# JuliaGaussianProcesses/ApproximateGPs.jl

Hardware: AMD Instinct MI355X
Metric: SVGP ELBO evals/sec at N=1e6, M=1024 (higher is better)
Workload: dtype f64

## Files before the change

### approximategps.jl_amd/csrc/device_common.hpp

```cpp
#pragma once
#include <hip/hip_runtime.h>
#include <type_traits>
#include <utility>

#include "diag.hpp"
#include <stdint.h>

#include <mutex>
#include <string>
#include <vector>

namespace svgp {

inline std::string& note_text() { static thread_local std::string s; return s; }
inline void leave_note(const std::string& s) {
  if (note_text().size() < 2048) note_text() += (note_text().empty() ? "" : "; ") + s;
}
inline std::string take_note() {
  std::string s;
  s.swap(note_text());
  return s;
}

inline void set_max_lds(const void* fn, hipFuncAttribute attr, int bytes) {
// ... 530 lines not shown
#endif
  using LdsP = const volatile __attribute__((address_space(3))) T*;
  struct RFrag { LdsP a, b0, b1; };
  static __device__ __forceinline__ LdsP lds_opaque(const T* p) {
    uint32_t v = uint32_t(uintptr_t((const __attribute__((address_space(3))) T*)(p)));
    asm("" : "+v"(v));
    return (LdsP)(uintptr_t(v));
  }
  static __device__ __forceinline__ RFrag rfrag(const T* smem) {
    const AFrag fr = afrag(smem);
    return RFrag{lds_opaque(fr.a), lds_opaque(fr.b0), lds_opaque(fr.b1)};
  }
  static constexpr int kMaxRotImmP = ((NBUF - 1) * PA_TILE + (kPairP ? 3 * 2 * PPP : 3 * 4 * PLD) + (MI - 1) * 32) * int(sizeof(T));
  static constexpr int kMaxRotImmQ = ((NBUF - 1) * QA_TILE + 3 * QSLAB + (NJ - 2) * 16) * int(sizeof(T));
  static_assert(!kAsync || (kMaxRotImmP < 65536 && kMaxRotImmQ < 65536), "a fragment read's offset must fit the ds_read immediate");
  template <int B, int KSLAB, int ILO = 0, int IHI = MI - 1>
  static __device__ __forceinline__ void load_rfrag(Frag& f, const RFrag& fr) {
    constexpr int AOFF = B * PA_TILE + (kPairP ? KSLAB * 2 * PPP : KSLAB * 4 * PLD);
    constexpr int QOFF = B * QA_TILE + KSLAB * QSLAB;
#pragma unroll
    for (int i = 0; i < MI; ++i)
      if (i >= ILO && i <= IHI) f.a[i] = fr.a[AOFF + i * 32];
    if (ILO <= IHI) {
      static_assert(NJ % 2 == 0, "column tiles come in even / odd pairs");
      static_assert(QR == 2 || NJ == 2, "the quad image is written for two column tiles per wave");
#pragma unroll
      for (int j = 0; j < NJ; j += 2) {
        f.b[j] = fr.b0[QOFF + j * 16];
        f.b[j + 1] = fr.b1[QOFF + j * 16];
      }
    }
  }
  struct ADst { uint32_t p, q; };
  static __device__ __forceinline__ ADst a_dst(const T* smem, int wv) {
    const uint32_t l = uint32_t(uintptr_t((const __attribute__((address_space(3))) T*)(smem)));
    return ADst{l + uint32_t(wv * (kPairP ? PPP : PLD) * int(sizeof(T))),
                l + uint32_t((NBUF * PA_TILE + wv * QPP) * int(sizeof(T)))};
  }
  template <int IMM>
  static __device__ __forceinline__ void glds16_at(const void* sbase, uint32_t voff, uint32_t lds) {
    asm volatile("s_add_u32 m0, %0, %3\n\tglobal_load_lds_dwordx4 %1, %2" ::"s"(lds), "v"(voff), "s"(sbase), "n"(IMM) : "memory", "scc");
  }
  template <int B>
  static __device__ __forceinline__ void dma_tile_at(const T* __restrict__ psrc, const T* __restrict__ qsrc, const AOff& off,
                                                     const ADst& dst) {
    if constexpr (!diag::ablate<1>) dma_rows<B * PA_TILE, NW * (kPairP ? PPP : PLD)>(psrc, off.p, dst.p, std::make_integer_sequence<int, DP>{});
    if constexpr (!diag::ablate<2>) dma_rows<B * QA_TILE, NW * QPP>(qsrc, off.q, dst.q, std::make_integer_sequence<int, DQ>{});
  }
  template <int BASE, int STRIDE, int N, int... Q>
  static __device__ __forceinline__ void dma_rows(const T* __restrict__ src, const uint32_t (&voff)[N], uint32_t dst,
                                                  std::integer_sequence<int, Q...>) {
    (glds16_at<(BASE + Q * STRIDE) * int(sizeof(T))>(src, voff[Q], dst), ...);
  }
  static constexpr int kAskT = -1;
  template <int B, int ILO, int IHI, int MORE = kAskT, typename QSrc, typename WSrc>
  static __device__ __forceinline__ void rstep(Acc& acc, Frag (&f)[2], const T* __restrict__ Pbase, int64_t pstride,
                                               const AOff& off, int t, int nsteps, QSrc& qsrc, WSrc& wsrc, T* __restrict__ smem,
                                               const ADst& dst, const RFrag& fr) {
    constexpr int KS = BK / 4;
    constexpr bool W = WSrc::on;
    constexpr int PER_TILE = DMA_PER_TILE + (W ? 1 : 0);
    constexpr int BN = (B + 1) % NBUF;
    static_assert(KS == 4, "written for 16-deep steps");
    static_assert(B >= 0 && B < NBUF, "buffer index");
    T* Ws = smem + NBUF * (PA_TILE + QA_TILE);
    const T* wl = Ws + B * W_TILE + ((threadIdx.x & 63) >> 4);
    load_rfrag<B, 1, ILO, IHI>(f[1], fr);
    mma_frag<ILO, IHI>(acc, f[0]);
    scale_b<1, W>(f[1], wl);
    load_rfrag<B, 2, ILO, IHI>(f[0], fr);
    mma_frag<ILO, IHI>(acc, f[1]);
    scale_b<2, W>(f[0], wl);
    load_rfrag<B, 3, ILO, IHI>(f[1], fr);
    mma_frag<ILO, IHI>(acc, f[0]);
    scale_b<3, W>(f[1], wl);
    const bool more1 = (MORE == kAskT) ? (t + 1 < nsteps) : (MORE >= 1);
    const bool more2 = (MORE == kAskT) ? (t + 2 < nsteps) : (MORE >= 2);
    const bool more3 = (MORE == kAskT) ? (t + 3 < nsteps) : (MORE >= 3);
    if (more1) {
      if (more2) wait_barrier<PER_TILE>();
      else wait_barrier<0>();
      load_rfrag<BN, 0>(f[0], fr);
      scale_b<0, W>(f[0], Ws + BN * W_TILE + ((threadIdx.x & 63) >> 4));
      if (more3) {
        dma_tile_at<B>(Pbase + int64_t(t + 3) * pstride, qsrc(t + 3), off, dst);
        if constexpr (W) dma_w(wsrc(t + 3), Ws + B * W_TILE);
      }
    }
    mma_frag<ILO, IHI>(acc, f[1]);
  }
#ifndef SVGP_WSTEP
#define SVGP_WSTEP 0
#endif
  struct WRegs { T w[4]; };
  static __device__ __forceinline__ void load_w(WRegs& wr, const T* __restrict__ wl) {
#pragma unroll
    for (int q = 0; q < 4; ++q) wr.w[q] = wl[q * 4];
  }
  template <int KSLAB>
  static __device__ __forceinline__ void scale_bw(Frag& f, const WRegs& wr) {
#pragma unroll
    for (int j = 0; j < NJ; ++j) f.b[j] *= wr.w[KSLAB];
  }
  template <typename QSrc, typename WSrc>
  static __device__ __forceinline__ void astep_w(Acc& acc, Frag (&f)[2], WRegs& wr, const T* __restrict__ Pbase, int64_t pstride,
                                                 const AOff& off, int t, int nsteps, QSrc& qsrc, WSrc& wsrc, T* __restrict__ smem,
                                                 int& b, const AFrag& fr) {
    constexpr int PER_TILE = DMA_PER_TILE + 1;
    static_assert(BK / 4 == 4, "written for 16-deep steps");
    const T* fa = fr.a + b * PA_TILE;
    const T* fb0 = fr.b0 + b * QA_TILE;
    const T* fb1 = fr.b1 + b * QA_TILE;
    T* Ws = smem + NBUF * (PA_TILE + QA_TILE);
    load_afrag<1>(f[1], fa, fb0, fb1);
    mma_frag(acc, f[0]);
    scale_bw<1>(f[1], wr);
    load_afrag<2>(f[0], fa, fb0, fb1);
    mma_frag(acc, f[1]);
    scale_bw<2>(f[0], wr);
    load_afrag<3>(f[1], fa, fb0, fb1);
    mma_frag(acc, f[0]);
    scale_bw<3>(f[1], wr);
    if (t + 1 < nsteps) {
      if (t + 2 < nsteps) wait_barrier<PER_TILE>();
      else wait_barrier<0>();
      const int bn = (b + 1 == NBUF) ? 0 : b + 1;
      load_w(wr, Ws + bn * W_TILE + ((threadIdx.x & 63) >> 4));
      load_afrag<0>(f[0], fr.a + bn * PA_TILE, fr.b0 + bn * QA_TILE, fr.b1 + bn * QA_TILE);
      if (t + 3 < nsteps) {
        dma_tile(Pbase + int64_t(t + 3) * pstride, qsrc(t + 3), off, smem + b * PA_TILE, smem + NBUF * PA_TILE + b * QA_TILE);
        dma_w(wsrc(t + 3), Ws + b * W_TILE);
      }
      b = bn;
      mma_frag(acc, f[1]);
#ifndef SVGP_WSTEP
#define SVGP_WSTEP 1
#endif
#if SVGP_WSTEP == 1
      __builtin_amdgcn_sched_barrier(0);
#endif
      scale_bw<0>(f[0], wr);
    } else {
      mma_frag(acc, f[1]);
    }
  }
#define SVGP_ASTEP(LO, HI, TT) astep<LO, HI>(acc, f, Pbase, pstride, off, (TT), nsteps, qsrc, wsrc, smem, b, fr)
#define SVGP_RSTEP(B, LO, HI, TT, ...) rstep<B, LO, HI, ##__VA_ARGS__>(acc, f, Pbase, pstride, off, (TT), nsteps, qsrc, wsrc, smem, dst, fr)
  template <int TRI, typename QSrc>
  static __device__ __forceinline__ void loop_tri_async(Acc& acc, const T* __restrict__ Pbase, int64_t ldp, int nsteps,
                                                        QSrc&& qsrc, T* __restrict__ smem, int64_t ldq = NT) {
    NoWeights nw;
    loop_tri_async_w<TRI>(acc, Pbase, ldp, nsteps, qsrc, nw, smem, ldq);
  }
  template <int TRI, typename QSrc, typename WSrc>
  static __device__ __forceinline__ void loop_tri_async_w(Acc& acc, const T* __restrict__ Pbase, int64_t ldp, int nsteps,
                                                          QSrc&& qsrc, WSrc&& wsrc, T* __restrict__ smem, int64_t ldq = NT) {
    if (nsteps <= 0) return;
    constexpr int ND = NB / BK;
    constexpr bool W = std::remove_reference_t<WSrc>::on;
    constexpr int PER_TILE = DMA_PER_TILE + (W ? 1 : 0);
    static_assert(TRI == 0 || (ND == 8 && MI == 4), "triangular steps are written out for BK = 16, 128-row panels");
    const AOff off = a_offsets(ldp, ldq);
    const int64_t pstride = int64_t(BK) * ldp;
    const int nreg = (TRI > 0) ? nsteps - ND : nsteps;
    Frag f[2];
    constexpr bool kTwin = W && TRI == 0 && SVGP_WSTEP != 0;
    if constexpr (SVGP_ASYNC_ROT && !kTwin) {
      constexpr bool kRemFirst = TRI >= 0;
      const int rem = kRemFirst ? nreg % NBUF : 0;
      const int s0 = (rem == 0) ? 0 : NBUF - rem, s1 = (s0 + 1 == NBUF) ? 0 : s0 + 1, s2 = (s1 + 1 == NBUF) ? 0 : s1 + 1;
      const ADst dst = a_dst(smem, wave_index());
      auto displaced = [&](int sb) { return ADst{dst.p + uint32_t(sb * PA_TILE * int(sizeof(T))), dst.q + uint32_t(sb * QA_TILE * int(sizeof(T)))}; };
      T* Ws = smem + NBUF * (PA_TILE + QA_TILE);
      dma_tile_at<0>(Pbase, qsrc(0), off, displaced(s0));
      if constexpr (W) dma_w(wsrc(0), Ws + s0 * W_TILE);
      if (nsteps > 1) {
        dma_tile_at<0>(Pbase + pstride, qsrc(1), off, displaced(s1));
        if constexpr (W) dma_w(wsrc(1), Ws + s1 * W_TILE);
      }
      if (nsteps > 2) {
        dma_tile_at<0>(Pbase + 2 * pstride, qsrc(2), off, displaced(s2));
        if constexpr (W) dma_w(wsrc(2), Ws + s2 * W_TILE);
      }
      if (nsteps > 2) wait_barrier<2 * PER_TILE>();
      else if (nsteps > 1) wait_barrier<PER_TILE>();
      else wait_barrier<0>();
      const RFrag fr = rfrag(smem);
      const T* wl0 = Ws + ((threadIdx.x & 63) >> 4);
      if constexpr (kRemFirst) {
        int zt = 0;
        asm volatile("" : "+s"(zt));
        int t = rem;
        if (rem == 0) {
          load_rfrag<0, 0>(f[0], fr);
          scale_b<0, W>(f[0], wl0);
        } else if (rem == 1) {
          load_rfrag<2, 0>(f[0], fr);
          scale_b<0, W>(f[0], wl0 + 2 * W_TILE);
          SVGP_RSTEP(2, 0, MI - 1, zt);
        } else {
          load_rfrag<1, 0>(f[0], fr);
          scale_b<0, W>(f[0], wl0 + W_TILE);
          SVGP_RSTEP(1, 0, MI - 1, zt); SVGP_RSTEP(2, 0, MI - 1, zt + 1);
        }
        for (; t < nreg; t += 3) {
          SVGP_RSTEP(0, 0, MI - 1, t); SVGP_RSTEP(1, 0, MI - 1, t + 1); SVGP_RSTEP(2, 0, MI - 1, t + 2);
        }
        if constexpr (TRI > 0) {
          SVGP_RSTEP(0, 0, 3, t + 0, 3); SVGP_RSTEP(1, 0, 3, t + 1, 3); SVGP_RSTEP(2, 1, 3, t + 2, 3); SVGP_RSTEP(0, 1, 3, t + 3, 3);
          SVGP_RSTEP(1, 2, 3, t + 4, 3); SVGP_RSTEP(2, 2, 3, t + 5, 2); SVGP_RSTEP(0, 3, 3, t + 6, 1); SVGP_RSTEP(1, 3, 3, t + 7, 0);
        }
      } else {
        load_rfrag<0, 0>(f[0], fr);
        scale_b<0, W>(f[0], wl0);
        SVGP_RSTEP(0, 0, 0, 0); SVGP_RSTEP(1, 0, 0, 1); SVGP_RSTEP(2, 0, 1, 2); SVGP_RSTEP(0, 0, 1, 3);
        SVGP_RSTEP(1, 0, 2, 4); SVGP_RSTEP(2, 0, 2, 5); SVGP_RSTEP(0, 0, 3, 6); SVGP_RSTEP(1, 0, 3, 7);
        constexpr int B0 = ND % NBUF, B1 = (B0 + 1) % NBUF, B2 = (B0 + 2) % NBUF;
        int t = ND;
        for (; t + 2 < nreg; t += 3) {
          SVGP_RSTEP(B0, 0, MI - 1, t); SVGP_RSTEP(B1, 0, MI - 1, t + 1); SVGP_RSTEP(B2, 0, MI - 1, t + 2);
        }
        if (t < nreg) SVGP_RSTEP(B0, 0, MI - 1, t);
        if (t + 1 < nreg) SVGP_RSTEP(B1, 0, MI - 1, t + 1);
      }
      __builtin_amdgcn_sched_barrier(0);
    } else {
      const AFrag fr = afrag(smem);
      T* Qs = smem + NBUF * PA_TILE;
      T* Ws = smem + NBUF * (PA_TILE + QA_TILE);
      dma_tile(Pbase, qsrc(0), off, smem, Qs);
      if constexpr (W) dma_w(wsrc(0), Ws);
      if (nsteps > 1) {
        dma_tile(Pbase + pstride, qsrc(1), off, smem + PA_TILE, Qs + QA_TILE);
        if constexpr (W) dma_w(wsrc(1), Ws + W_TILE);
      }
      if (nsteps > 2) {
        dma_tile(Pbase + 2 * pstride, qsrc(2), off, smem + 2 * PA_TILE, Qs + 2 * QA_TILE);
        if constexpr (W) dma_w(wsrc(2), Ws + 2 * W_TILE);
      }
      if (nsteps > 2) wait_barrier<2 * PER_TILE>();
      else if (nsteps > 1) wait_barrier<PER_TILE>();
      else wait_barrier<0>();
      load_afrag<0>(f[0], fr.a, fr.b0, fr.b1);
      scale_b<0, W>(f[0], Ws + ((threadIdx.x & 63) >> 4));
      int b = 0, t = 0;
      if (TRI < 0) {
        SVGP_ASTEP(0, 0, 0); SVGP_ASTEP(0, 0, 1); SVGP_ASTEP(0, 1, 2); SVGP_ASTEP(0, 1, 3);
        SVGP_ASTEP(0, 2, 4); SVGP_ASTEP(0, 2, 5); SVGP_ASTEP(0, 3, 6); SVGP_ASTEP(0, 3, 7);
        t = ND;
      }
      if constexpr (kTwin) {
        WRegs wr;
        load_w(wr, Ws + ((threadIdx.x & 63) >> 4));
        for (; t < nreg; ++t) astep_w(acc, f, wr, Pbase, pstride, off, t, nsteps, qsrc, wsrc, smem, b, fr);
      } else {
        for (; t < nreg; ++t) astep<0, MI - 1>(acc, f, Pbase, pstride, off, t, nsteps, qsrc, wsrc, smem, b, fr);
      }
      if (TRI > 0) {
        SVGP_ASTEP(0, 3, nreg + 0); SVGP_ASTEP(0, 3, nreg + 1); SVGP_ASTEP(1, 3, nreg + 2); SVGP_ASTEP(1, 3, nreg + 3);
        SVGP_ASTEP(2, 3, nreg + 4); SVGP_ASTEP(2, 3, nreg + 5); SVGP_ASTEP(3, 3, nreg + 6); SVGP_ASTEP(3, 3, nreg + 7);
      }
    }
    __syncthreads();
  }
#undef SVGP_RSTEP
#undef SVGP_ASTEP
};

}
```

### approximategps.jl_amd/csrc/diag.hpp

```cpp
#pragma once
#include <hip/hip_runtime.h>

namespace svgp {
namespace diag {
#ifdef SVGP_ABLATE
constexpr int kAblate = SVGP_ABLATE;
#else
constexpr int kAblate = 0;
#endif
template <int BIT>
inline constexpr bool ablate = (kAblate & BIT) != 0;
}
}

#if defined(SVGP_STRIP_STAMPS) && defined(SVGP_DIAG_TU_STRIP)
namespace svgp {
__device__ unsigned long long g_strip_stamps[128];
__shared__ unsigned long long s_strip_stamps[128];
__device__ unsigned long long g_wg_times[16][12];
}
extern "C" int svgp_debug_strip_stamps(unsigned long long* out) {
  return int(hipMemcpyFromSymbol(out, HIP_SYMBOL(svgp::g_strip_stamps), sizeof(svgp::g_strip_stamps)));
}
extern "C" int svgp_debug_wg_times(unsigned long long* out) {
  return int(hipMemcpyFromSymbol(out, HIP_SYMBOL(svgp::g_wg_times), sizeof(svgp::g_wg_times)));
}
#define SVGP_SSTAMP(i) do { if (stamping && threadIdx.x == 0) s_strip_stamps[i] += clock64(); } while (0)
#define SVGP_SSTAMP_KERNEL_BEGIN()                            \
  int strips_done = 0;                                        \
  if (threadIdx.x < 128) s_strip_stamps[threadIdx.x] = 0;     \
  __syncthreads()
#define SVGP_SSTAMP_STRIP_BEGIN()                                                                                          \
  const bool stamping = (blockIdx.x == 37 && strips_done >= 1);                                                            \
  if (stamping && threadIdx.x == 0) s_strip_stamps[127] += 1;                                                              \
  if (threadIdx.x == 0 && blockIdx.x % 37 == 0 && blockIdx.x / 37 < 16 && strips_done < 10)                                \
    g_wg_times[blockIdx.x / 37][strips_done] = clock64();                                                                  \
  ++strips_done
#define SVGP_SSTAMP_KERNEL_END()                                                                                           \
  do {                                                                                                                     \
    if (blockIdx.x == 37 && threadIdx.x < 128) g_strip_stamps[threadIdx.x] = s_strip_stamps[threadIdx.x];                  \
    if (threadIdx.x == 0 && blockIdx.x % 37 == 0 && blockIdx.x / 37 < 16) {                                                \
      g_wg_times[blockIdx.x / 37][10] = clock64();                                                                         \
      g_wg_times[blockIdx.x / 37][11] = (unsigned long long)(__builtin_amdgcn_s_getreg((20 << 0) | (0 << 6) | (3 << 11)) & 0xf) | \
                                        ((unsigned long long)strips_done << 8);                         \
      for (int q = strips_done; q < 10; ++q) g_wg_times[blockIdx.x / 37][q] = 0;                                           \
    }                                                                                                                      \
  } while (0)
#else
#define SVGP_SSTAMP(i)
#define SVGP_SSTAMP_KERNEL_BEGIN()
#define SVGP_SSTAMP_STRIP_BEGIN()
#define SVGP_SSTAMP_KERNEL_END()
#endif

#if defined(SVGP_POTF2_STAMPS) && defined(SVGP_DIAG_TU_PREP)
namespace svgp {
__device__ unsigned long long g_potf2_stamps[128];
}
extern "C" int svgp_debug_potf2_stamps(unsigned long long* out) {
  return int(hipMemcpyFromSymbol(out, HIP_SYMBOL(svgp::g_potf2_stamps), sizeof(svgp::g_potf2_stamps)));
}
#define SVGP_STAMP(i) do { if (threadIdx.x == 0) g_potf2_stamps[i] = clock64(); } while (0)
#define SVGP_STAMPW(i) do { if (threadIdx.x == 64) g_potf2_stamps[i] = clock64(); } while (0)
#else
#define SVGP_STAMP(i)
#define SVGP_STAMPW(i)
#endif
```

### approximategps.jl_amd/csrc/strip.hip

```cpp
#define SVGP_DIAG_TU_STRIP
#include "device_common.hpp"
#include "kernels.hpp"
#include "knobs.hpp"
#include "lik.hpp"

#ifndef SVGP_ASYNC
#define SVGP_ASYNC 1
#endif
#ifndef SVGP_TRI
#define SVGP_TRI 3
#endif

#include <cstdlib>
#include <type_traits>

namespace svgp {

namespace {

#ifndef SVGP_PREGEN_EXPTAB
#define SVGP_PREGEN_EXPTAB 1
#endif
template <typename T, int NT, int NTHR, int F, int DL>
__device__ __forceinline__ void pregen_mfma(const T* __restrict__ xs, const T* __restrict__ zs, int d, int64_t Mp, int64_t M,
                                            double variance_d, T* __restrict__ work, const double* __restrict__ exptab = nullptr) {
  constexpr int KS = DL / 4, JT = NT / 16, NW = NTHR / 64;
  constexpr bool XREG = (DL <= 16);
  using M16 = Mfma16<T>;
  using acc_t = typename M16::acc_t;
  const int lane = threadIdx.x & 63, wave = threadIdx.x >> 6, l15 = lane & 15, g = lane >> 4;
  const T variance = T(variance_d);
  const T c1 = (F == KSE) ? T(-0.5) : T(1);
  const T c0 = (F == KSE) ? T(log(variance_d)) : T(0);
  const T ascale = (F == KSE) ? T(1) : T(-2);
  T xb[XREG ? JT : 1][XREG ? KS : 1], xn[JT];
  const T* __restrict__ xl = xs + g * NT + l15;
#pragma unroll
  for (int jt = 0; jt < JT; ++jt) {
    T s = T(0);
#pragma unroll
    for (int q = 0; q < KS; ++q) {
      const T v = xl[(4 * q) * NT + jt * 16];
      if constexpr (XREG) xb[jt][q] = v;
      s = fma(v, v, s);
    }
    s += __shfl_xor(s, 16);
    s += __shfl_xor(s, 32);
    xn[jt] = fma(c1, s, c0);
  }
  for (int kb = wave; kb < int(Mp / 16); kb += NW) {
    const int64_t k0 = int64_t(kb) * 16;
    const bool inside = __builtin_amdgcn_readfirstlane(int(k0 + 16 <= M)) != 0;
    T za[KS];
    T s = T(0);
#pragma unroll
    for (int q = 0; q < KS; ++q) {
      const int f = 4 * q + g;
      const T v = (f < d) ? zs[int64_t(f) * Mp + k0 + l15] : T(0);
      za[q] = ascale * v;
      s = fma(v, v, s);
    }
    s += __shfl_xor(s, 16);
    s += __shfl_xor(s, 32);
    s *= c1;
    T zn[4];
#pragma unroll
    for (int r = 0; r < 4; ++r) zn[r] = __shfl(s, M16::row(lane, r));
#pragma unroll
    for (int jt = 0; jt < JT; ++jt) {
      acc_t acc;
#pragma unroll
      for (int r = 0; r < 4; ++r) acc[r] = xn[jt] + zn[r];
      if constexpr (XREG) {
#pragma unroll
        for (int q = 0; q < KS; ++q) acc = M16::mma(za[q], xb[jt][q], acc);
      } else {
        acc_t acc2 = {0, 0, 0, 0};
        __builtin_amdgcn_sched_barrier(0);
#pragma unroll
        for (int q = 0; q < KS; q += 2) {
          acc = M16::mma(za[q], xl[(4 * q) * NT + jt * 16], acc);
          acc2 = M16::mma(za[q + 1], xl[(4 * q + 4) * NT + jt * 16], acc2);
        }
#pragma unroll
        for (int r = 0; r < 4; ++r) acc[r] += acc2[r];
      }
      T out[4];
#pragma unroll
      for (int r = 0; r < 4; ++r) {
        const T v = acc[r];
        if constexpr (SVGP_PREGEN_EXPTAB && F == KSE && sizeof(T) == 8) out[r] = T(kexp_tab(double(v > c0 ? c0 : v), exptab));
        else out[r] = (F == KSE) ? kexp(v > c0 ? c0 : v) : kappa<T>(F, v < T(0) ? T(0) : v, variance);
      }
      if (inside) {
#pragma unroll
        for (int r = 0; r < 4; ++r) work[(k0 + M16::row(lane, r)) * NT + jt * 16 + l15] = out[r];
      } else {
#pragma unroll
        for (int r = 0; r < 4; ++r) {
          const int64_t k = k0 + M16::row(lane, r);
          work[k * NT + jt * 16 + l15] = (k < M) ? out[r] : T(0);
        }
        asm volatile("" ::: "memory");
      }
    }
  }
}


template <typename G, typename T, int NT, int NTHR>
__device__ __forceinline__ void store_tile_point_major(const typename G::Acc& acc, T* __restrict__ smem, T* __restrict__ out,
                                                       int64_t c0, int64_t Mp, int row0) {
  constexpr int HC = NT < 64 ? NT : 64, RS = G::NB + (sizeof(T) == 8 ? 4 : 8), VEC = G::VEC, CPR = G::NB / VEC;
  using V = typename G::V;
  static_assert(size_t(HC) * RS * sizeof(T) <= ((SVGP_ASYNC && G::kAsync) ? G::ASYNC_LDS_BYTES : G::LDS_BYTES),
                "the transposition tile must fit the staging buffers");
#pragma unroll
  for (int p = 0; p < NT / HC; ++p) {
#pragma unroll
    for (int j = 0; j < G::NJ; ++j) {
      const int col = G::acc_col(j);
      if (col / HC == p) {
#pragma unroll
        for (int i = 0; i < G::MI; ++i)
#pragma unroll
          for (int r = 0; r < 4; ++r) smem[(col % HC) * RS + G::acc_row(i, r)] = acc.v[i][j][r];
      }
    }
    __syncthreads();
    for (int e = threadIdx.x; e < HC * CPR; e += NTHR) {
      const int col = e / CPR, rv = (e % CPR) * VEC;
      *reinterpret_cast<V*>(out + (c0 + p * HC + col) * Mp + row0 + rv) = *reinterpret_cast<const V*>(smem + col * RS + rv);
    }
    __syncthreads();
  }
}

#ifndef SVGP_STRIP_PRIO
#define SVGP_STRIP_PRIO 1
#endif
template <bool ON>
__device__ __forceinline__ void strip_prio(int strips_done) {
  if constexpr (ON && SVGP_STRIP_PRIO != 0) {
    if ((strips_done + (blockIdx.x >= gridDim.x / 2 ? 1 : 0)) & 1) __builtin_amdgcn_s_setprio(0);
    else __builtin_amdgcn_s_setprio(1);
  }
}

struct PointGrads { double e, gmu, gv, gs2; };
__device__ __noinline__ PointGrads strip_point_grads(LikParams lp, double mu, double v, double yv, double scale) {
  double a = 0.0, b = 0.0, gs2 = 0.0;
  expected_loglik_grad_point(lp, mu, v, yv, a, b, gs2);
  PointGrads r;
  r.e = expected_loglik_point(lp, mu, v, yv, log(lp.sigma2));
  r.gmu = a * scale;
  r.gv = b * scale;
  r.gs2 = gs2 * scale;
  return r;
}

template <typename T, int NT, int BK, int NTHR, int MINW = 2, int PAD = 16, bool GRAD = false, bool BIGD = false, bool SEG = false>
__global__ void __launch_bounds__(NTHR, MINW) strip_kernel(StripArgs a, int64_t nstrips) {
  using G = TileGemm<T, NT, BK, NTHR, PAD>;
  using Acc = typename G::Acc;
  using QRegs = typename G::QRegs;
  constexpr int NB = G::NB, MI = G::MI, NJ = G::NJ, VEC = G::VEC;

  extern __shared__ __attribute__((aligned(16))) unsigned char smem_raw[];
  T* smem = reinterpret_cast<T*>(smem_raw);
  T* xs = smem;
  const int pre_dl = BIGD ? (a.kp.d <= 32 ? 32 : 64) : (a.kp.d <= 8 ? 8 : a.kp.d <= 16 ? 16 : 0);
  const int dl = pre_dl ? pre_dl : a.kp.d;

  const T* __restrict__ Tm = static_cast<const T*>(a.T);
  const T* __restrict__ U = static_cast<const T*>(a.U);
  const T* __restrict__ zs = static_cast<const T*>(a.zs);
  const T* __restrict__ mp = static_cast<const T*>(a.mp);
  const T* __restrict__ x = static_cast<const T*>(a.x);
  const T* __restrict__ invl = static_cast<const T*>(a.kp.invl);
  const int64_t Mp = a.Mp, M = a.M;
  const int d = a.kp.d, family = a.kp.family;
  const T variance = T(a.kp.variance);
  const int nP = int(Mp / NB);
  T* __restrict__ work = static_cast<T*>(a.work) + int64_t(blockIdx.x) * Mp * NT;
  T* __restrict__ workK = (GRAD && !diag::ablate<256>) ? static_cast<T*>(a.work) + (int64_t(gridDim.x) + blockIdx.x) * Mp * NT : work;
  const int tid = threadIdx.x, lane = tid & 63;
  const typename G::QOff qoff = G::q_offsets(NT);

  __shared__ unsigned next_strip;
#if SVGP_PREGEN_EXPTAB
  __shared__ double s_exptab[64];
  if (sizeof(T) == 8 && threadIdx.x < 64) s_exptab[threadIdx.x] = exp2(double(threadIdx.x) * 0.015625);
  const double* exptab = s_exptab;
#else
  const double* exptab = nullptr;
#endif
  SVGP_SSTAMP_KERNEL_BEGIN();
  [[maybe_unused]] int prio_strips = 0;
  [[maybe_unused]] int part = 0, nsplit = 1;
  if constexpr (SEG) {
    if (a.seg_split > 1) { nsplit = a.seg_split; part = int(blockIdx.x / nstrips); }
  }
  for (int64_t strip = (nsplit > 1) ? int64_t(blockIdx.x % nstrips) : int64_t(blockIdx.x); strip < nstrips;) {
    if constexpr (SEG) {
      work = static_cast<T*>(a.work) + strip * Mp * NT;
      workK = GRAD ? static_cast<T*>(a.work) + (nstrips + strip) * Mp * NT : work;
    }
    SVGP_SSTAMP_STRIP_BEGIN();
    SVGP_SSTAMP(0);
    strip_prio<GRAD && !SEG>(prio_strips++);
    const int64_t c0 = strip * NT;
    if constexpr (SEG) { if (tid == 0) next_strip = unsigned(strip + gridDim.x); }
    else if (tid == 0) next_strip = gridDim.x + atomicAdd(a.counter, 1u);
    const int64_t last = a.off + a.len - 1;
    const bool do_pregen = !SEG || (a.seg_flags & kSegPregen);
    if (do_pregen)
    for (int e = tid; e < dl * NT; e += NTHR) {
      const int f = e / NT, c = e % NT;
      int64_t g = a.off + c0 + c;
      g = g > last ? last : g;
      xs[e] = (f < d) ? x[int64_t(f) * a.ldx + g] * invl[f] : T(0);
    }
    __syncthreads();
    if (do_pregen) {
      auto pregen = [&](auto fam) {
        constexpr int F = decltype(fam)::value;
        using V = typename G::V;
        constexpr int CPR = NT / VEC;
        for (int e = tid; e < int(Mp) * CPR; e += NTHR) {
          const int k = e / CPR, c = (e % CPR) * VEC;
          T r2[VEC];
#pragma unroll
          for (int q = 0; q < VEC; ++q) r2[q] = T(0);
#pragma unroll 8
          for (int f = 0; f < d; ++f) {
            const T zf = zs[int64_t(f) * Mp + k];
            const V xf = *reinterpret_cast<const V*>(xs + f * NT + c);
#pragma unroll
            for (int q = 0; q < VEC; ++q) {
              const T df = xf[q] - zf;
              r2[q] = fma(df, df, r2[q]);
            }
          }
          V out;
#pragma unroll
          for (int q = 0; q < VEC; ++q) out[q] = (k < M) ? kappa<T>(F, r2[q], variance) : T(0);
          *reinterpret_cast<V*>(workK + int64_t(k) * NT + c) = out;
        }
      };
      if constexpr (BIGD) {
        if (pre_dl == 32) {
          if (family == KSE) pregen_mfma<T, NT, NTHR, KSE, 32>(xs, zs, d, Mp, M, a.kp.variance, workK, exptab);
          else if (family == KM32) pregen_mfma<T, NT, NTHR, KM32, 32>(xs, zs, d, Mp, M, a.kp.variance, workK);
          else pregen_mfma<T, NT, NTHR, KM52, 32>(xs, zs, d, Mp, M, a.kp.variance, workK);
        } else {
          if (family == KSE) pregen_mfma<T, NT, NTHR, KSE, 64>(xs, zs, d, Mp, M, a.kp.variance, workK, exptab);
          else if (family == KM32) pregen_mfma<T, NT, NTHR, KM32, 64>(xs, zs, d, Mp, M, a.kp.variance, workK);
          else pregen_mfma<T, NT, NTHR, KM52, 64>(xs, zs, d, Mp, M, a.kp.variance, workK);
        }
      } else if (pre_dl == 8) {
        if (family == KSE) pregen_mfma<T, NT, NTHR, KSE, 8>(xs, zs, d, Mp, M, a.kp.variance, workK, exptab);
        else if (family == KM32) pregen_mfma<T, NT, NTHR, KM32, 8>(xs, zs, d, Mp, M, a.kp.variance, workK);
        else pregen_mfma<T, NT, NTHR, KM52, 8>(xs, zs, d, Mp, M, a.kp.variance, workK);
      } else if (pre_dl == 16) {
        if (family == KSE) pregen_mfma<T, NT, NTHR, KSE, 16>(xs, zs, d, Mp, M, a.kp.variance, workK, exptab);
        else if (family == KM32) pregen_mfma<T, NT, NTHR, KM32, 16>(xs, zs, d, Mp, M, a.kp.variance, workK);
        else pregen_mfma<T, NT, NTHR, KM52, 16>(xs, zs, d, Mp, M, a.kp.variance, workK);
      } else if (family == KSE) pregen(std::integral_constant<int, KSE>{});
      else if (family == KM32) pregen(std::integral_constant<int, KM32>{});
      else pregen(std::integral_constant<int, KM52>{});
      __syncthreads();
    }

    double sA[NJ], sM[NJ], sC[NJ];
#pragma unroll
    for (int j = 0; j < NJ; ++j) sA[j] = sM[j] = sC[j] = 0.0;
    int I_lo = 0, I_hi = nP;
    if constexpr (SEG) {
      I_lo = a.seg_lo;
      I_hi = a.seg_hi;
      if ((a.seg_flags & kSegLoad) && part == 0) {
        const double* __restrict__ st = a.seg_state + (strip * NTHR + tid) * (2 * NJ);
#pragma unroll
        for (int j = 0; j < NJ; ++j) { sA[j] = st[j]; sM[j] = st[NJ + j]; }
      }
    }

    SVGP_SSTAMP(1);
    for (int I = I_lo; I < I_hi; ++I) {
      SVGP_SSTAMP(2 + 3 * I);
      Acc acc;
      acc.zero();
      const int tK = I * (NB / BK);
      if constexpr (SVGP_ASYNC && G::kAsync) {
        auto qsrc = [&](int t) { return (t < tK ? work : workK) + int64_t(t) * BK * NT; };
        G::template loop_tri_async<(SVGP_TRI & 1) ? 1 : 0>(acc, Tm + int64_t(I) * NB, Mp, (I + 1) * (NB / BK), qsrc, smem);
      } else {
        auto qload = [&](int t, QRegs& r) { G::load_q(r, (t < tK ? work : workK) + int64_t(t) * BK * NT, qoff); };
        G::template loop_tri<(BK == 16 && (SVGP_TRI & 1)) ? 1 : 0>(acc, Tm + int64_t(I) * NB, Mp, (I + 1) * (NB / BK), qload, smem);
      }

      SVGP_SSTAMP(3 + 3 * I);
#pragma unroll
      for (int i = 0; i < MI; ++i) {
#pragma unroll
        for (int r = 0; r < 4; ++r) {
          const int row = I * NB + G::acc_row(i, r);
          const double mr = double(mp[row]);
#pragma unroll
          for (int j = 0; j < NJ; ++j) {
            const T val = acc.v[i][j][r];
            const int col = G::acc_col(j);
            if constexpr (!diag::ablate<4>) work[int64_t(row) * NT + col] = val;
            if (a.A_out) static_cast<T*>(a.A_out)[int64_t(row) * a.lda + c0 + col] = val;
            if constexpr (!GRAD) {
              if (a.At_out) static_cast<T*>(a.At_out)[(c0 + col) * Mp + row] = val;
            }
            if constexpr (!diag::ablate<16>) {
              const double dv = double(val);
              if constexpr (!GRAD) sA[j] = fma(dv, dv, sA[j]);
              sM[j] = fma(dv, mr, sM[j]);
            } else {
              sA[j] += double(val) + mr;
            }
          }
        }
      }
      if constexpr (GRAD && !diag::ablate<32>) store_tile_point_major<G, T, NT, NTHR>(acc, smem, static_cast<T*>(a.At_out), c0, Mp, I * NB);
      __syncthreads();
      SVGP_SSTAMP(4 + 3 * I);
    }

    if constexpr (SEG) {
      if (a.seg_flags & kSegStore) {
        double* __restrict__ st = a.seg_state + (strip * NTHR + tid) * (2 * NJ);
#pragma unroll
        for (int j = 0; j < NJ; ++j) { st[j] = sA[j]; st[NJ + j] = sM[j]; }
      }
      if (!(a.seg_flags & kSegPhase2)) {
        strip = next_strip;
        __syncthreads();
        continue;
      }
    }
    if constexpr (!GRAD)
    for (int J = SEG ? part : 0; J < nP; J += (SEG ? nsplit : 1)) {
      SVGP_SSTAMP(60 + 2 * J);
      Acc acc;
      acc.zero();
      const T* wq = work + int64_t(J) * NB * NT;
      if constexpr (SVGP_ASYNC && G::kAsync) {
        auto qsrc = [&](int t) { return wq + int64_t(t) * BK * NT; };
        G::template loop_tri_async<(SVGP_TRI & 2) ? -1 : 0>(acc, U + int64_t(J) * NB + int64_t(J) * NB * Mp, Mp, (nP - J) * (NB / BK), qsrc,
                                                            smem);
      } else {
        auto qload = [&](int t, QRegs& r) { G::load_q(r, wq + int64_t(t) * BK * NT, qoff); };
        G::template loop_tri<(BK == 16 && (SVGP_TRI & 2)) ? -1 : 0>(acc, U + int64_t(J) * NB + int64_t(J) * NB * Mp, Mp, (nP - J) * (NB / BK), qload,
                                                   smem);
      }
      SVGP_SSTAMP(61 + 2 * J);
#pragma unroll
      for (int i = 0; i < MI; ++i)
#pragma unroll
        for (int r = 0; r < 4; ++r)
#pragma unroll
          for (int j = 0; j < NJ; ++j) {
            const T val = acc.v[i][j][r];
            if (a.C_out) static_cast<T*>(a.C_out)[int64_t(J * NB + G::acc_row(i, r)) * a.lda + c0 + G::acc_col(j)] = val;
            if (a.Ct_out) static_cast<T*>(a.Ct_out)[(c0 + G::acc_col(j)) * Mp + J * NB + G::acc_row(i, r)] = val;
            const double dv = double(val);
            sC[j] = fma(dv, dv, sC[j]);
          }
    }

    if constexpr (GRAD) {
      const T* __restrict__ Rm = static_cast<const T*>(a.R);
      T* __restrict__ Pt = static_cast<T*>(a.Pt_out);
      int p3_lo = 0, p3_hi = nP;
      if constexpr (SEG) { p3_lo = (part * nP) / nsplit; p3_hi = ((part + 1) * nP) / nsplit; }
      for (int I = p3_lo; I < p3_hi; ++I) {
        SVGP_SSTAMP(26 + 4 * I);
        Acc acc;
        acc.zero();
        if constexpr (SVGP_ASYNC && G::kAsync) {
          auto qsrc = [&](int t) { return work + int64_t(t) * BK * NT; };
          G::template loop_tri_async<0>(acc, Rm + int64_t(I) * NB, Mp, nP * (NB / BK), qsrc, smem);
        } else {
          auto qload = [&](int t, QRegs& r) { G::load_q(r, work + int64_t(t) * BK * NT, qoff); };
          G::template loop_tri<0>(acc, Rm + int64_t(I) * NB, Mp, nP * (NB / BK), qload, smem);
        }
        SVGP_SSTAMP(27 + 4 * I);
        if constexpr (!diag::ablate<128>) {
#pragma unroll
          for (int i = 0; i < MI; ++i)
#pragma unroll
            for (int r = 0; r < 4; ++r) {
              const int64_t row = int64_t(I) * NB + G::acc_row(i, r);
#pragma unroll
              for (int j = 0; j < NJ; ++j) sC[j] = fma(double(acc.v[i][j][r]), double(workK[row * NT + G::acc_col(j)]), sC[j]);
            }
        } else {
#pragma unroll
          for (int j = 0; j < NJ; ++j) sC[j] += double(acc.v[0][j][0]);
        }
        SVGP_SSTAMP(28 + 4 * I);
        if constexpr (!diag::ablate<64>) store_tile_point_major<G, T, NT, NTHR>(acc, smem, Pt, c0, Mp, I * NB);
        else if (acc.v[0][0][0] == T(12345.678)) Pt[c0] = acc.v[0][0][0];
        SVGP_SSTAMP(29 + 4 * I);
      }
    }

    SVGP_SSTAMP(100);
    double* red = reinterpret_cast<double*>(smem_raw);
#pragma unroll
    for (int j = 0; j < NJ; ++j) {
      double va = sA[j], vm = sM[j], vc = sC[j];
      va += __shfl_xor(va, 16); va += __shfl_xor(va, 32);
      vm += __shfl_xor(vm, 16); vm += __shfl_xor(vm, 32);
      vc += __shfl_xor(vc, 16); vc += __shfl_xor(vc, 32);
      if ((lane >> 4) == 0) {
        const int wr = (tid >> 6) / G::WC;
        const int col = G::acc_col(j);
        red[(0 * G::WR + wr) * NT + col] = va;
        red[(1 * G::WR + wr) * NT + col] = vm;
        red[(2 * G::WR + wr) * NT + col] = vc;
      }
    }
    __syncthreads();
    {
      bool split_done = false;
      if constexpr (SEG) {
        if (nsplit > 1) {
          __shared__ int s_last_part;
          if (tid < NT) {
            double qa = 0, qm = 0, qc = 0;
#pragma unroll
            for (int w = 0; w < G::WR; ++w) {
              qa += red[(0 * G::WR + w) * NT + tid];
              qm += red[(1 * G::WR + w) * NT + tid];
              qc += red[(2 * G::WR + w) * NT + tid];
            }
            double* __restrict__ pp = a.seg_part + ((int64_t(part) * nstrips + strip) * 3) * NT;
            pp[tid] = qa;
            pp[NT + tid] = qm;
            pp[2 * NT + tid] = qc;
          }
          __threadfence();
          __syncthreads();
          if (tid == 0) s_last_part = (__hip_atomic_fetch_add(&a.seg_cnt[strip], 1u, __ATOMIC_ACQ_REL, __HIP_MEMORY_SCOPE_AGENT) == unsigned(nsplit - 1));
          __syncthreads();
          if (s_last_part) {
            __threadfence();
            if (tid < NT && c0 + tid < a.len) {
              double qa = 0, qm = 0, qc = 0;
              for (int q = 0; q < nsplit; ++q) {
                const double* __restrict__ pp = a.seg_part + ((int64_t(q) * nstrips + strip) * 3) * NT;
                qa += __builtin_nontemporal_load(pp + tid);
                qm += __builtin_nontemporal_load(pp + NT + tid);
                qc += __builtin_nontemporal_load(pp + 2 * NT + tid);
              }
              const double mc = a.mux ? a.mean_const + double(static_cast<const T*>(a.mux)[c0 + tid]) : a.mean_const;
              a.mom_mu[c0 + tid] = mc + qm;
              a.mom_var[c0 + tid] = a.kp.variance - qa + qc;
            }
          }
          __syncthreads();
          split_done = true;
        }
      }
      if (!split_done) {
      if (tid < NT && c0 + tid < a.len) {
        double qa = 0, qm = 0, qc = 0;
#pragma unroll
        for (int w = 0; w < G::WR; ++w) {
          qa += red[(0 * G::WR + w) * NT + tid];
          qm += red[(1 * G::WR + w) * NT + tid];
          qc += red[(2 * G::WR + w) * NT + tid];
        }
        const double mc = a.mux ? a.mean_const + double(static_cast<const T*>(a.mux)[c0 + tid]) : a.mean_const;
        a.mom_mu[c0 + tid] = mc + qm;
        a.mom_var[c0 + tid] = a.kp.variance - qa + qc;
      }
      __syncthreads();
      }
    }
    strip = next_strip;
    __syncthreads();
    SVGP_SSTAMP(101);
  }
  SVGP_SSTAMP_KERNEL_END();
}

template <typename T, int NT, int BK, int NTHR, int MINW = 2, int PAD = 16, bool BIGD = false>
__global__ void __launch_bounds__(NTHR, MINW) trsm_pm_kernel(StripArgs a, int64_t nstrips) {
  using G = TileGemm<T, NT, BK, NTHR, PAD>;
  using Acc = typename G::Acc;
  using QRegs = typename G::QRegs;
  constexpr int NB = G::NB, MI = G::MI, NJ = G::NJ;

  extern __shared__ __attribute__((aligned(16))) unsigned char smem_raw[];
  T* smem = reinterpret_cast<T*>(smem_raw);
  T* xs = smem;
  const int pre_dl = BIGD ? (a.kp.d <= 32 ? 32 : 64) : (a.kp.d <= 8 ? 8 : 16);
  const T* __restrict__ Tm = static_cast<const T*>(a.T);
  const T* __restrict__ zs = static_cast<const T*>(a.zs);
  const T* __restrict__ x = static_cast<const T*>(a.x);
  const T* __restrict__ invl = static_cast<const T*>(a.kp.invl);
  const int64_t Mp = a.Mp, M = a.M;
  const int d = a.kp.d, family = a.kp.family;
  const int nP = int(Mp / NB);
  T* __restrict__ work = static_cast<T*>(a.work) + int64_t(blockIdx.x) * Mp * NT;
  const int tid = threadIdx.x, lane = tid & 63;
  [[maybe_unused]] const typename G::QOff qoff = G::q_offsets(NT);
// ... 729 lines not shown
```

Measured before the change: 31.19.

## Prefetch next panel's first tiles during epilogue of current panel

Adds a cross-panel prefetch for the strip kernel's triangular async loops. After each panel's accumulation finishes, the first three tiles of the next panel (or the first U panel) are issued via async DMA into the rotation buffers before the epilogue stores, and the next loop entry skips its own prologue loads and only waits. The goal is to hide the loop-prologue load latency behind the epilogue write-out. In exchange the buffer-slot choice must agree exactly between prefetch and loop, and the first-panel Q source is assumed to come from work (tK=0). Timing stamps for loop entry are also added.

```diff
diff --git a/approximategps.jl_amd/csrc/device_common.hpp b/approximategps.jl_amd/csrc/device_common.hpp
--- a/approximategps.jl_amd/csrc/device_common.hpp
+++ b/approximategps.jl_amd/csrc/device_common.hpp
@@ -706,9 +706,40 @@
     NoWeights nw;
     loop_tri_async_w<TRI>(acc, Pbase, ldp, nsteps, qsrc, nw, smem, ldq);
   }
-  template <int TRI, typename QSrc, typename WSrc>
+#ifndef SVGP_XPANEL
+#define SVGP_XPANEL 1
+#endif
+  template <int TRI>
+  static __device__ __forceinline__ int rot_rem(int nsteps) {
+    return (TRI >= 0) ? ((TRI > 0) ? nsteps - NB / BK : nsteps) % NBUF : 0;
+  }
+  template <int TRI, typename QSrc>
+  static __device__ __forceinline__ void prefetch_tri_async(const T* __restrict__ Pbase, int64_t ldp, int nsteps, QSrc&& qsrc,
+                                                            T* __restrict__ smem, int64_t ldq = NT) {
+    static_assert(SVGP_ASYNC_ROT != 0, "written for the compile-time rotation");
+    if (nsteps <= 0) return;
+    const AOff off = a_offsets(ldp, ldq);
+    const int64_t pstride = int64_t(BK) * ldp;
+    const int rem = rot_rem<TRI>(nsteps);
+    const int s0 = (rem == 0) ? 0 : NBUF - rem, s1 = (s0 + 1 == NBUF) ? 0 : s0 + 1, s2 = (s1 + 1 == NBUF) ? 0 : s1 + 1;
+    const ADst dst = a_dst(smem, wave_index());
+    auto displaced = [&](int sb) { return ADst{dst.p + uint32_t(sb * PA_TILE * int(sizeof(T))), dst.q + uint32_t(sb * QA_TILE * int(sizeof(T)))}; };
+    int zt = 0;
+    asm volatile("" : "+s"(zt));
+    dma_tile_at<0>(Pbase + int64_t(zt) * pstride, qsrc(zt), off, displaced(s0));
+    if (nsteps > 1) dma_tile_at<0>(Pbase + int64_t(zt + 1) * pstride, qsrc(zt + 1), off, displaced(s1));
+    if (nsteps > 2) dma_tile_at<0>(Pbase + int64_t(zt + 2) * pstride, qsrc(zt + 2), off, displaced(s2));
+  }
+  template <int TRI, typename QSrc>
+  static __device__ __forceinline__ void loop_tri_async_pre(Acc& acc, const T* __restrict__ Pbase, int64_t ldp, int nsteps,
+                                                            QSrc&& qsrc, T* __restrict__ smem, bool prefetched, int64_t ldq = NT) {
+    NoWeights nw;
+    loop_tri_async_w<TRI, QSrc&, NoWeights&, true>(acc, Pbase, ldp, nsteps, qsrc, nw, smem, ldq, prefetched);
+  }
+  template <int TRI, typename QSrc, typename WSrc, bool PRE = false>
   static __device__ __forceinline__ void loop_tri_async_w(Acc& acc, const T* __restrict__ Pbase, int64_t ldp, int nsteps,
-                                                          QSrc&& qsrc, WSrc&& wsrc, T* __restrict__ smem, int64_t ldq = NT) {
+                                                          QSrc&& qsrc, WSrc&& wsrc, T* __restrict__ smem, int64_t ldq = NT,
+                                                          [[maybe_unused]] bool prefetched = false) {
     if (nsteps <= 0) return;
     constexpr int ND = NB / BK;
     constexpr bool W = std::remove_reference_t<WSrc>::on;
@@ -719,6 +750,7 @@
     const int nreg = (TRI > 0) ? nsteps - ND : nsteps;
     Frag f[2];
     constexpr bool kTwin = W && TRI == 0 && SVGP_WSTEP != 0;
+    static_assert(!PRE || (SVGP_ASYNC_ROT != 0 && !kTwin), "the prefetched entry exists on the compile-time rotation only");
     if constexpr (SVGP_ASYNC_ROT && !kTwin) {
       constexpr bool kRemFirst = TRI >= 0;
       const int rem = kRemFirst ? nreg % NBUF : 0;
@@ -726,19 +758,27 @@
       const ADst dst = a_dst(smem, wave_index());
       auto displaced = [&](int sb) { return ADst{dst.p + uint32_t(sb * PA_TILE * int(sizeof(T))), dst.q + uint32_t(sb * QA_TILE * int(sizeof(T)))}; };
       T* Ws = smem + NBUF * (PA_TILE + QA_TILE);
-      dma_tile_at<0>(Pbase, qsrc(0), off, displaced(s0));
-      if constexpr (W) dma_w(wsrc(0), Ws + s0 * W_TILE);
-      if (nsteps > 1) {
-        dma_tile_at<0>(Pbase + pstride, qsrc(1), off, displaced(s1));
-        if constexpr (W) dma_w(wsrc(1), Ws + s1 * W_TILE);
-      }
-      if (nsteps > 2) {
-        dma_tile_at<0>(Pbase + 2 * pstride, qsrc(2), off, displaced(s2));
-        if constexpr (W) dma_w(wsrc(2), Ws + s2 * W_TILE);
-      }
-      if (nsteps > 2) wait_barrier<2 * PER_TILE>();
-      else if (nsteps > 1) wait_barrier<PER_TILE>();
-      else wait_barrier<0>();
+      static_assert(!PRE || !W, "the prefetch carries no weights");
+      bool issued = false;
+      if constexpr (PRE) issued = prefetched;
+      if (issued) {
+        wait_barrier<0>();
+      } else {
+        dma_tile_at<0>(Pbase, qsrc(0), off, displaced(s0));
+        if constexpr (W) dma_w(wsrc(0), Ws + s0 * W_TILE);
+        if (nsteps > 1) {
+          dma_tile_at<0>(Pbase + pstride, qsrc(1), off, displaced(s1));
+          if constexpr (W) dma_w(wsrc(1), Ws + s1 * W_TILE);
+        }
+        if (nsteps > 2) {
+          dma_tile_at<0>(Pbase + 2 * pstride, qsrc(2), off, displaced(s2));
+          if constexpr (W) dma_w(wsrc(2), Ws + s2 * W_TILE);
+        }
+        if (nsteps > 2) wait_barrier<2 * PER_TILE>();
+        else if (nsteps > 1) wait_barrier<PER_TILE>();
+        else wait_barrier<0>();
+      }
+      SVGP_SSTAMP_LOOP_ENTRY();
       const RFrag fr = rfrag(smem);
       const T* wl0 = Ws + ((threadIdx.x & 63) >> 4);
       if constexpr (kRemFirst) {
diff --git a/approximategps.jl_amd/csrc/diag.hpp b/approximategps.jl_amd/csrc/diag.hpp
--- a/approximategps.jl_amd/csrc/diag.hpp
+++ b/approximategps.jl_amd/csrc/diag.hpp
@@ -26,6 +26,9 @@
   return int(hipMemcpyFromSymbol(out, HIP_SYMBOL(svgp::g_wg_times), sizeof(svgp::g_wg_times)));
 }
 #define SVGP_SSTAMP(i) do { if (stamping && threadIdx.x == 0) s_strip_stamps[i] += clock64(); } while (0)
+__shared__ unsigned long long s_loop_entry;
+#define SVGP_SSTAMP_LOOP_ENTRY() do { if (threadIdx.x == 0) s_loop_entry = clock64(); } while (0)
+#define SVGP_SSTAMP_ENTRY(i) do { if (stamping && threadIdx.x == 0) s_strip_stamps[i] += s_loop_entry; } while (0)
 #define SVGP_SSTAMP_KERNEL_BEGIN()                            \
   int strips_done = 0;                                        \
   if (threadIdx.x < 128) s_strip_stamps[threadIdx.x] = 0;     \
@@ -48,6 +51,8 @@
   } while (0)
 #else
 #define SVGP_SSTAMP(i)
+#define SVGP_SSTAMP_LOOP_ENTRY()
+#define SVGP_SSTAMP_ENTRY(i)
 #define SVGP_SSTAMP_KERNEL_BEGIN()
 #define SVGP_SSTAMP_STRIP_BEGIN()
 #define SVGP_SSTAMP_KERNEL_END()
diff --git a/approximategps.jl_amd/csrc/strip.hip b/approximategps.jl_amd/csrc/strip.hip
--- a/approximategps.jl_amd/csrc/strip.hip
+++ b/approximategps.jl_amd/csrc/strip.hip
@@ -165,6 +165,7 @@
   using Acc = typename G::Acc;
   using QRegs = typename G::QRegs;
   constexpr int NB = G::NB, MI = G::MI, NJ = G::NJ, VEC = G::VEC;
+  constexpr bool kXPanel = SVGP_XPANEL && SVGP_ASYNC && SVGP_ASYNC_ROT && G::kAsync && !GRAD && !SEG;
 
   extern __shared__ __attribute__((aligned(16))) unsigned char smem_raw[];
   T* smem = reinterpret_cast<T*>(smem_raw);
@@ -275,6 +276,7 @@
     double sA[NJ], sM[NJ], sC[NJ];
 #pragma unroll
     for (int j = 0; j < NJ; ++j) sA[j] = sM[j] = sC[j] = 0.0;
+    [[maybe_unused]] bool prefetched = false;
     int I_lo = 0, I_hi = nP;
     if constexpr (SEG) {
       I_lo = a.seg_lo;
@@ -292,7 +294,10 @@
       Acc acc;
       acc.zero();
       const int tK = I * (NB / BK);
-      if constexpr (SVGP_ASYNC && G::kAsync) {
+      if constexpr (kXPanel) {
+        auto qsrc = [&](int t) { return (t < tK ? work : workK) + int64_t(t) * BK * NT; };
+        G::template loop_tri_async_pre<(SVGP_TRI & 1) ? 1 : 0>(acc, Tm + int64_t(I) * NB, Mp, (I + 1) * (NB / BK), qsrc, smem, prefetched);
+      } else if constexpr (SVGP_ASYNC && G::kAsync) {
         auto qsrc = [&](int t) { return (t < tK ? work : workK) + int64_t(t) * BK * NT; };
         G::template loop_tri_async<(SVGP_TRI & 1) ? 1 : 0>(acc, Tm + int64_t(I) * NB, Mp, (I + 1) * (NB / BK), qsrc, smem);
       } else {
@@ -301,6 +306,15 @@
       }
 
       SVGP_SSTAMP(3 + 3 * I);
+      SVGP_SSTAMP_ENTRY(102 + I);
+      if constexpr (kXPanel) {
+        prefetched = (I >= 1);
+        if (prefetched) {
+          auto qhead = [&](int t) { return work + int64_t(t) * BK * NT; };
+          if (I + 1 < nP) G::template prefetch_tri_async<(SVGP_TRI & 1) ? 1 : 0>(Tm + int64_t(I + 1) * NB, Mp, (I + 2) * (NB / BK), qhead, smem);
+          else G::template prefetch_tri_async<(SVGP_TRI & 2) ? -1 : 0>(U, Mp, nP * (NB / BK), qhead, smem);
+        }
+      }
 #pragma unroll
       for (int i = 0; i < MI; ++i) {
 #pragma unroll
@@ -349,7 +363,11 @@
       Acc acc;
       acc.zero();
       const T* wq = work + int64_t(J) * NB * NT;
-      if constexpr (SVGP_ASYNC && G::kAsync) {
+      if constexpr (kXPanel) {
+        auto qsrc = [&](int t) { return wq + int64_t(t) * BK * NT; };
+        G::template loop_tri_async_pre<(SVGP_TRI & 2) ? -1 : 0>(acc, U + int64_t(J) * NB + int64_t(J) * NB * Mp, Mp, (nP - J) * (NB / BK), qsrc,
+                                                                smem, prefetched);
+      } else if constexpr (SVGP_ASYNC && G::kAsync) {
         auto qsrc = [&](int t) { return wq + int64_t(t) * BK * NT; };
         G::template loop_tri_async<(SVGP_TRI & 2) ? -1 : 0>(acc, U + int64_t(J) * NB + int64_t(J) * NB * Mp, Mp, (nP - J) * (NB / BK), qsrc,
                                                             smem);
@@ -359,6 +377,15 @@
                                                    smem);
       }
       SVGP_SSTAMP(61 + 2 * J);
+      SVGP_SSTAMP_ENTRY(110 + J);
+      if constexpr (kXPanel) {
+        prefetched = (J + 1 < nP);
+        if (prefetched) {
+          auto qnext = [&](int t) { return wq + int64_t(NB + t * BK) * NT; };
+          G::template prefetch_tri_async<(SVGP_TRI & 2) ? -1 : 0>(U + int64_t(J + 1) * NB + int64_t(J + 1) * NB * Mp, Mp, (nP - J - 1) * (NB / BK),
+                                                                  qnext, smem);
+        }
+      }
 #pragma unroll
       for (int i = 0; i < MI; ++i)
 #pragma unroll
```

New measurement: 31.17. Within noise of the previous version (-0.1%).
